# udaysankar01/xfeatSLAM

Measured on AMD Instinct MI355X. Metric: XFeat frames/s (VGA, 4096 kpts) + 4096x4096 desc-match pairs/s, higher is better.
Workload: dtype f32

## Files before the change

### xfeatslam_amd/csrc/kernels_conv.hip

```cpp
#include "ctx.h"
#include "heads_kp4.hip.h"
#include <stdlib.h>

struct ConvArgs {
    const float* in;
    StatSrc st;
    size_t in_stride;
    int Hin, Win;
    const float* w;
    const float* bias;
    float* out;
    size_t out_stride;
    int Hout, Wout;
    double* part;
    size_t part_stride;
    int tiles_x;
    const float* pool; size_t pool_stride; const float* skip_w; const float* skip_b;
    const float* r4; size_t s4; int H4, W4; StatSrc st4;
    const float* r5; size_t s5; int H5, W5; StatSrc st5;
    const float* xstat; const float* w0; const float* bias0;
    int dbg;
};

enum { PRO_PLAIN = 0, PRO_BN = 1, PRO_IN = 2, PRO_B2IN = 3, PRO_FUSE = 4, PRO_L0 = 5, PRO_UNFOLD = 6, PRO_FUSEA = 7  };
// ... 364 lines not shown
                                              int rows_left, int cols_left, int co0, int h, const float (&bias)[NT] ,
                                              double (&sum)[NT], double (&sq)[NT]) {
    static_assert(WW >= 8 && WW * WH == 32, "pixel block of a wave");
    XFH_MFMA_SETTLE();
    const bool full = rows_left >= WH && cols_left >= WW;
    const int lane_off = 4 * h * COUT + co0;
    const int rowstride = Wout * COUT;
    auto value = [&](int n, int r, float* dst, float bv) {
        float v = acc[n][r];
        if constexpr (EPI != EPI_STATS) v += bv;
        if constexpr (EPI == EPI_BIAS_RELU) v = fmaxf(v, 0.f);
        dst[lane_off] = v;
        if constexpr (EPI == EPI_STATS) { const double dv = (double)v; sum[n] += dv; sq[n] = fma(dv, dv, sq[n]); }
    };
    if (full) {
#pragma unroll
        for (int n = 0; n < NT; ++n) {
            sum[n] = 0.0; sq[n] = 0.0;
            if (COUT % 32 == 0 || co0 + n * 32 < COUT) {
#pragma unroll
                for (int r = 0; r < 16; ++r) {
                    const int pb = (r & 3) + 8 * (r >> 2);
                    value(n, r, wave_out + (pb / WW) * rowstride + (pb % WW) * COUT + n * 32, bias[n]);
                }
            }
        }
        return;
    }
#pragma unroll
    for (int n = 0; n < NT; ++n) {
        const int co = co0 + n * 32;
        sum[n] = 0.0; sq[n] = 0.0;
        const float bv = bias[n];
        const bool cok = COUT % 32 == 0 || co < COUT;
#pragma unroll
        for (int r = 0; r < 16; ++r) {
            const int pb = (r & 3) + 8 * (r >> 2);
            const int prow = pb / WW, pcol = pb % WW;
            float* dst = wave_out + prow * rowstride + pcol * COUT + n * 32;
            if (cok && prow < rows_left && pcol + 4 * h < cols_left) value(n, r, dst, bv);
        }
    }
}

#ifndef XFH_PD
#define XFH_PD 3
#endif

template <int CIN, int COUT, int KS, int ST, int WM, int WN, int NT, int WW, int PRO, int EPI, int CBMAX = 64, int TPC = 1, int PD = XFH_PD>
__device__ __forceinline__ void conv_mfma_body(const ConvArgs a, const int tile, const int b, float* smem) {
    constexpr int NTHR = 64 * WM * WN;
    constexpr int WH = 32 / WW, TH = WM * WH, TW = WW;
    constexpr int COUTP = WN * NT * 32;
    constexpr int PAD = KS / 2;
    constexpr int TIH = (TH - 1) * ST + KS, TIW = (TW - 1) * ST + KS;
    constexpr int CP = CIN + 4;
    constexpr int CB = CIN > CBMAX ? CBMAX : CIN;
    constexpr int NCB = CIN / CB;
    static_assert(TPC == 1 || NCB == 1, "several taps per chunk only with all channels in the chunk");
    static_assert((KS * KS) % TPC == 0, "taps per chunk");
    constexpr int NCHUNK = KS * KS * NCB / TPC;
    constexpr int NWBUF = NCHUNK > 1 ? 2 : 1;
    constexpr int KC = TPC * CB;
    constexpr int WS = KC + 4;
    constexpr int WCH = COUTP * KC;
    constexpr int NWLD = (WCH / 4 + NTHR - 1) / NTHR;
    constexpr int G = CIN / 8;
    constexpr int IN_FLOATS = TIH * TIW * CP;
    constexpr int W_FLOATS = COUTP * WS;

    float* s_in = smem;
    float* s_w = smem + IN_FLOATS;
    float* s_stat = s_w + NWBUF * W_FLOATS;

    const int t = threadIdx.x;
    const int tx0 = (tile % a.tiles_x) * TW, ty0 = (tile / a.tiles_x) * TH;
    const float* in = a.in + (size_t)b * a.in_stride;

    XFH_STAMP(a, 0);
    f32x4 wreg[PD][NWLD];
    const __amdgpu_buffer_rsrc_t wrs = wbuf_make(a.w);
#pragma unroll
    for (int c = 0; c < PD; ++c)
#pragma unroll
        for (int q = 0; q < NWLD; ++q) {
            const int f = t + q * NTHR;
            if (c < NCHUNK && f < WCH / 4) wreg[c][q] = wbuf_ld(wrs, f, c * WCH);
        }
    constexpr int NITEM = TIH * TIW * G;
    constexpr int NIT = (NITEM + NTHR - 1) / NTHR;
    constexpr bool FUSE = PRO == PRO_FUSE || PRO == PRO_FUSEA;
    constexpr bool BATCHED = !FUSE;
    f32x4 r0[BATCHED ? NIT : 1], r1[BATCHED ? NIT : 1];
    float rp[PRO == PRO_B2IN ? NIT : 1];
    if constexpr (BATCHED) {
#pragma unroll
        for (int k = 0; k < NIT; ++k) {
            const int item = t + k * NTHR, pix = item / G, g = item % G;
            const int gy = min(max(ty0 * ST - PAD + pix / TIW, 0), a.Hin - 1), gx = min(max(tx0 * ST - PAD + pix % TIW, 0), a.Win - 1);
            const float* p = PRO == PRO_UNFOLD ? in + ((size_t)(gy * 8 + g) * (a.Win * 8) + gx * 8) : in + ((size_t)gy * a.Win + gx) * CIN + g * 8;
            r0[k] = *(const f32x4*)p;
            r1[k] = *(const f32x4*)(p + 4);
            if constexpr (PRO == PRO_B2IN) rp[k] = a.pool[(size_t)b * a.pool_stride + (size_t)gy * a.Win + gx];
        }
    }
    XFH_STAMP(a, 1);
    if constexpr (PRO == PRO_BN || PRO == PRO_B2IN || FUSE) stage_stat(a.st, b, CIN, tile == 0, s_stat, (double*)s_in, t, NTHR);
    if constexpr (PRO == PRO_B2IN) {
        for (int q = t; q < CIN; q += NTHR) { s_stat[2 * CIN + q] = a.skip_w[q]; s_stat[3 * CIN + q] = a.skip_b[q]; }
        __syncthreads();
    }
    if constexpr (PRO == PRO_FUSE) {
        stage_stat(a.st4, b, 64, tile == 0, s_stat + 128, (double*)s_in, t, NTHR);
        stage_stat(a.st5, b, 64, tile == 0, s_stat + 256, (double*)s_in, t, NTHR);
    }
    XFH_STAMP(a, 2);
    if constexpr (BATCHED) {
#pragma unroll
        for (int k = 0; k < NIT; ++k) {
            const int item = t + k * NTHR, pix = item / G, g = item % G;
            const int gy = ty0 * ST - PAD + pix / TIW, gx = tx0 * ST - PAD + pix % TIW;
            const bool ok = gy >= 0 && gy < a.Hin && gx >= 0 && gx < a.Win;
            if (NITEM % NTHR != 0 && item >= NITEM) continue;
            f32x4 v0 = r0[k], v1 = r1[k];
            if constexpr (PRO == PRO_UNFOLD) {
                const float xm = a.xstat[b * 2], xr = a.xstat[b * 2 + 1];
#pragma unroll
                for (int q = 0; q < 4; ++q) { v0[q] = fmaf(v0[q], xr, xm); v1[q] = fmaf(v1[q], xr, xm); }
            }
            if constexpr (PRO == PRO_BN || PRO == PRO_B2IN) {
                const f32x4 m0 = *(const f32x4*)(s_stat + g * 8), m1 = *(const f32x4*)(s_stat + g * 8 + 4);
                const f32x4 q0 = *(const f32x4*)(s_stat + CIN + g * 8), q1 = *(const f32x4*)(s_stat + CIN + g * 8 + 4);
#pragma unroll
                for (int q = 0; q < 4; ++q) {
                    v0[q] = fmaxf(fmaf(v0[q], q0[q], m0[q]), 0.f);
                    v1[q] = fmaxf(fmaf(v1[q], q1[q], m1[q]), 0.f);
                }
            }
            if constexpr (PRO == PRO_B2IN) {
                const float pl = rp[k];
#pragma unroll
                for (int q = 0; q < 4; ++q) {
                    v0[q] = v0[q] + (pl * s_stat[2 * CIN + g * 8 + q] + s_stat[3 * CIN + g * 8 + q]);
                    v1[q] = v1[q] + (pl * s_stat[2 * CIN + g * 8 + 4 + q] + s_stat[3 * CIN + g * 8 + 4 + q]);
                }
            }
            if constexpr (KS > 1) { if (!ok) { v0 = f32x4{0.f, 0.f, 0.f, 0.f}; v1 = v0; } }
            float* d = s_in + pix * CP + g * 8;
            *(f32x4*)d = f32x4{v0.x, v0.z, v1.x, v1.z};
            *(f32x4*)(d + 4) = f32x4{v0.y, v0.w, v1.y, v1.w};
        }
    } else
    for (int item = t; item < TIH * TIW * G; item += NTHR) {
        const int pix = item / G, g = item % G;
        const int iy = pix / TIW, ix = pix % TIW;
        const int gy = ty0 * ST - PAD + iy, gx = tx0 * ST - PAD + ix;
        f32x4 v0 = {0.f, 0.f, 0.f, 0.f}, v1 = {0.f, 0.f, 0.f, 0.f};
        if (gy >= 0 && gy < a.Hin && gx >= 0 && gx < a.Win) {
            const float* p = in + ((size_t)gy * a.Win + gx) * CIN + g * 8;
            v0 = *(const f32x4*)p;
            v1 = *(const f32x4*)(p + 4);
#pragma unroll
            for (int q = 0; q < 4; ++q) {
                v0[q] = fmaxf(fmaf(v0[q], s_stat[CIN + g * 8 + q], s_stat[g * 8 + q]), 0.f);
                v1[q] = fmaxf(fmaf(v1[q], s_stat[CIN + g * 8 + 4 + q], s_stat[g * 8 + 4 + q]), 0.f);
            }
            f32x4 u0, u1, w0, w1;
            up_bilinear8<PRO == PRO_FUSEA>(a.r4 + (size_t)b * a.s4, s_stat + 128, a.H4, a.W4, a.Hin, a.Win, gy, gx, g, u0, u1);
            up_bilinear8<PRO == PRO_FUSEA>(a.r5 + (size_t)b * a.s5, s_stat + 256, a.H5, a.W5, a.Hin, a.Win, gy, gx, g, w0, w1);
#pragma unroll
            for (int q = 0; q < 4; ++q) { v0[q] = (v0[q] + u0[q]) + w0[q]; v1[q] = (v1[q] + u1[q]) + w1[q]; }
        }
        float* d = s_in + pix * CP + g * 8;
        *(f32x4*)d = f32x4{v0.x, v0.z, v1.x, v1.z};
        *(f32x4*)(d + 4) = f32x4{v0.y, v0.w, v1.y, v1.w};
    }
#pragma unroll
    for (int q = 0; q < NWLD; ++q) {
        const int f = t + q * NTHR;
        if (f < WCH / 4) {
            const int n = f / (KC / 4), c4 = f % (KC / 4);
            *(f32x4*)(s_w + n * WS + c4 * 4) = wreg[0][q];
            if (PD < NCHUNK) wreg[0][q] = wbuf_ld(wrs, f, PD * WCH);
        }
    }
    __syncthreads();
    XFH_STAMP(a, 3);

    const int wave = __builtin_amdgcn_readfirstlane(t >> 6), lane = t & 63, i = lane & 31, h = lane >> 5;
    const int wm = wave / WN, wn = wave % WN;
    const int pr = i / WW, pc = i % WW;
    const int ly = (wm * WH + pr) * ST, lx = pc * ST;

    float biasv[NT];
    conv_bias<COUT, NT, EPI>(a.bias, wn * NT * 32 + i, biasv);
    f32x16 acc[NT];
#pragma unroll
    for (int n = 0; n < NT; ++n)
#pragma unroll
        for (int r = 0; r < 16; ++r) acc[n][r] = 0.f;

#pragma unroll
    for (int ch = 0; ch < NCHUNK; ++ch) {
#pragma unroll
        for (int tt = 0; tt < TPC; ++tt) {
            const int tap = TPC == 1 ? ch / NCB : ch * TPC + tt, cb = TPC == 1 ? ch % NCB : 0;
            const int ky = tap / KS, kx = tap % KS;
            const float* pa = s_in + ((ly + ky) * TIW + lx + kx) * CP + cb * CB + 4 * h;
            const float* pw = s_w + (ch & 1) * W_FLOATS + (wn * NT * 32 + i) * WS + tt * CB + 4 * h;
#pragma unroll
            for (int kk = 0; kk < CB / 8; ++kk) {
                const f32x4 av = *(const f32x4*)(pa + kk * 8);
#pragma unroll
                for (int n = 0; n < NT; ++n) {
                    const f32x4 bv = *(const f32x4*)(pw + n * 32 * WS + kk * 8);
#pragma unroll
                    for (int j = 0; j < 4; ++j)
                        acc[n] = __builtin_amdgcn_mfma_f32_32x32x2f32(av[j], bv[j], acc[n], 0, 0, 0);
                }
            }
        }
        if (ch + 1 < NCHUNK) {
            float* wd = s_w + ((ch + 1) & 1) * W_FLOATS;
#pragma unroll
            for (int q = 0; q < NWLD; ++q) {
                const int f = t + q * NTHR;
                if (f < WCH / 4) {
                    const int n = f / (KC / 4), c4 = f % (KC / 4);
                    *(f32x4*)(wd + n * WS + c4 * 4) = wreg[(ch + 1) % PD][q];
                    if (ch + 1 + PD < NCHUNK) wreg[(ch + 1) % PD][q] = wbuf_ld(wrs, f, (ch + 1 + PD) * WCH);
                }
            }
        }
        __syncthreads();
    }

    XFH_STAMP(a, 4);
    double sum[NT], sq[NT];
    {
        const int oy0 = ty0 + wm * WH;
        float* wave_out = a.out + (size_t)b * a.out_stride + ((size_t)oy0 * a.Wout + tx0) * COUT;
        conv_epilogue<COUT, NT, WW, WH, EPI>(acc, wave_out, a.Wout, a.Hout - oy0, a.Wout - tx0, wn * NT * 32 + i, h, biasv, sum, sq);
    }
    if constexpr (EPI == EPI_STATS) {
        double* s_red = (double*)smem;
#pragma unroll
        for (int n = 0; n < NT; ++n) {
            sum[n] += __shfl_xor(sum[n], 32);
            sq[n] += __shfl_xor(sq[n], 32);
            if (h == 0) {
                const int co = (wn * NT + n) * 32 + i;
                s_red[(wm * COUTP + co) * 2 + 0] = sum[n];
                s_red[(wm * COUTP + co) * 2 + 1] = sq[n];
            }
        }
        __syncthreads();
        for (int co = t; co < COUT; co += NTHR) {
            double S = 0.0, SS = 0.0;
#pragma unroll
            for (int m = 0; m < WM; ++m) { S += s_red[(m * COUTP + co) * 2 + 0]; SS += s_red[(m * COUTP + co) * 2 + 1]; }
            double* p = a.part + (size_t)b * a.part_stride + ((size_t)tile * COUT + co) * 2;
            p[0] = S; p[1] = SS;
        }
    }
    XFH_STAMP(a, 5);
}

template <int CIN, int COUT, int KS, int ST, int WM, int WN, int NT, int WW, int PRO, int EPI, int CBMAX = 64, int TPC = 1, int PD = XFH_PD>
__global__ __launch_bounds__(64 * WM * WN)
void k_conv_mfma(ConvArgs a) {
    extern __shared__ __attribute__((aligned(16))) float smem[];
    conv_mfma_body<CIN, COUT, KS, ST, WM, WN, NT, WW, PRO, EPI, CBMAX, TPC, PD>(a, blockIdx.x, blockIdx.z, smem);
}

enum { RIDE_UNFOLD = 0 , RIDE_BN = 1 , RIDE_KP4 = 2  };
template <int CIN, int COUT, int KS, int ST, int WM, int WN, int NT, int WW, int PRO, int CBMAX, int TPC, int RIDER, int EPI = EPI_STATS>
__global__ __launch_bounds__(256)
void k_conv_mfma_ride(ConvArgs a, int n_host, ConvArgs r, Kp4Args k) {
    static_assert(WM * WN == 4, "256 threads");
    extern __shared__ __attribute__((aligned(16))) float smem[];
    const int blk = blockIdx.x;
    if (blk < n_host) conv_mfma_body<CIN, COUT, KS, ST, WM, WN, NT, WW, PRO, EPI, CBMAX, TPC>(a, blk, blockIdx.z, smem);
    else if constexpr (RIDER == RIDE_KP4) { if (threadIdx.x < 4 * HK4_PX) heads_kp4_body(k, blk - n_host, blockIdx.z, smem); }
    else conv_mfma_body<64, 64, 1, 1, 4, 1, 2, 16, RIDER == RIDE_UNFOLD ? PRO_UNFOLD : PRO_BN, EPI>(r, blk - n_host, blockIdx.z, smem);
}

template <int CIN, int COUT, int KS, int ST, int WM, int WN, int NT, int WW, int PRO, int EPI>
__global__ __launch_bounds__(64 * WM * WN)
void k_conv_mfma_p(ConvArgs a, int ntile, int total) {
    constexpr int NTHR = 64 * WM * WN;
    constexpr int WH = 32 / WW, TH = WM * WH, TW = WW;
    constexpr int COUTP = WN * NT * 32;
    constexpr int PAD = KS / 2;
    constexpr int TIH = (TH - 1) * ST + KS, TIW = (TW - 1) * ST + KS;
    constexpr int CP = CIN + 4;
    constexpr int KTOT = KS * KS * CIN;
    constexpr int WS = KTOT + 4;
    constexpr int G = CIN / 8;
    constexpr int NITEM = TIH * TIW * G;
    constexpr int NE = NTHR / G * G;
    constexpr int NIT = (NITEM + NE - 1) / NE;
    constexpr int IN_FLOATS = TIH * TIW * CP;
    constexpr int W_FLOATS = COUTP * WS;
    static_assert(NIT <= 32, "inside mask");

    extern __shared__ __attribute__((aligned(16))) float smem[];
    float* s_in = smem;
    float* s_w = smem + IN_FLOATS;
    double* s_red = (double*)(s_w + W_FLOATS);

    const int t = threadIdx.x;
    for (int f = t; f < COUTP * (KTOT / 4); f += NTHR) {
        const int n = f / (KTOT / 4), c4 = f % (KTOT / 4);
        *(f32x4*)(s_w + n * WS + c4 * 4) = *(const f32x4*)(a.w + (size_t)f * 4);
    }
    const int g = t % G;
    const int wave = __builtin_amdgcn_readfirstlane(t >> 6), lane = t & 63, i = lane & 31, h = lane >> 5;
    const int wm = wave / WN, wn = wave % WN;
    const int pr = i / WW, pc = i % WW;
    const int ly = (wm * WH + pr) * ST, lx = pc * ST;

    f32x4 v0[NIT], v1[NIT];
    float pl[NIT];
    unsigned inside = 0u;
    auto load_tile = [&](int tile) {
        const int b = tile / ntile, tl = tile - b * ntile;
        const int tx0 = (tl % a.tiles_x) * TW, ty0 = (tl / a.tiles_x) * TH;
        const float* in = a.in + (size_t)b * a.in_stride + (PRO == PRO_UNFOLD ? 0 : g * 8);
        inside = 0u;
#pragma unroll
        for (int k = 0; k < NIT; ++k) {
            const int item = t + k * NE;
            const int pix = item / G;
            const int iy = pix / TIW, ix = pix % TIW;
            const int gy = ty0 * ST - PAD + iy, gx = tx0 * ST - PAD + ix;
            if constexpr (KS == 1) {
                const int cy = min(max(gy, 0), a.Hin - 1), cx = min(max(gx, 0), a.Win - 1);
                const float* p = PRO == PRO_UNFOLD ? in + ((cy * 8 + g) * (a.Win * 8) + cx * 8) : in + (cy * a.Win + cx) * CIN;
                v0[k] = *(const f32x4*)p; v1[k] = *(const f32x4*)(p + 4);
            } else {
                v0[k] = f32x4{0.f, 0.f, 0.f, 0.f}; v1[k] = v0[k];
                if (t < NE && item < NITEM && gy >= 0 && gy < a.Hin && gx >= 0 && gx < a.Win) {
                    const float* p = in + (gy * a.Win + gx) * CIN;
                    v0[k] = *(const f32x4*)p; v1[k] = *(const f32x4*)(p + 4);
                    if constexpr (PRO == PRO_B2IN) pl[k] = a.pool[(size_t)b * a.pool_stride + (size_t)gy * a.Win + gx];
                    inside |= 1u << k;
                }
            }
        }
    };
    auto store_tile = [&](int tile) {
        f32x4 m0, m1, r0, r1, w0, w1, c0, c1;
        if constexpr (PRO == PRO_BN || PRO == PRO_B2IN) {
            const int b = tile / ntile;
            const float* st = a.st.stat + (size_t)b * 2 * CIN + g * 8;
            m0 = *(const f32x4*)st; m1 = *(const f32x4*)(st + 4); r0 = *(const f32x4*)(st + CIN); r1 = *(const f32x4*)(st + CIN + 4);
        }
        if constexpr (PRO == PRO_B2IN) {
            w0 = *(const f32x4*)(a.skip_w + g * 8); w1 = *(const f32x4*)(a.skip_w + g * 8 + 4);
            c0 = *(const f32x4*)(a.skip_b + g * 8); c1 = *(const f32x4*)(a.skip_b + g * 8 + 4);
        }
#pragma unroll
        for (int k = 0; k < NIT; ++k) {
            const int item = t + k * NE;
            if (t < NE && item < NITEM) {
                f32x4 x0 = v0[k], x1 = v1[k];
                [[maybe_unused]] const bool in_img = inside & (1u << k);
                if constexpr (KS == 1) {
                    float xm = 0.f, xr = 1.f;
                    if constexpr (PRO == PRO_UNFOLD) { const int fb = tile / ntile; xm = a.xstat[fb * 2]; xr = a.xstat[fb * 2 + 1]; }
#pragma unroll
                    for (int q = 0; q < 4; ++q) {
                        if constexpr (PRO == PRO_UNFOLD) { x0[q] = fmaf(x0[q], xr, xm); x1[q] = fmaf(x1[q], xr, xm); }
                        if constexpr (PRO == PRO_BN) {
                            x0[q] = fmaxf(fmaf(x0[q], r0[q], m0[q]), 0.f);
                            x1[q] = fmaxf(fmaf(x1[q], r1[q], m1[q]), 0.f);
                        }
                    }
                } else if constexpr (PRO == PRO_BN || PRO == PRO_B2IN) {
                    if (in_img) {
#pragma unroll
                        for (int q = 0; q < 4; ++q) {
                            x0[q] = fmaxf(fmaf(x0[q], r0[q], m0[q]), 0.f);
                            x1[q] = fmaxf(fmaf(x1[q], r1[q], m1[q]), 0.f);
                            if constexpr (PRO == PRO_B2IN) { x0[q] = x0[q] + (pl[k] * w0[q] + c0[q]); x1[q] = x1[q] + (pl[k] * w1[q] + c1[q]); }
                        }
                    }
                }
                float* d = s_in + (item / G) * CP + g * 8;
                *(f32x4*)d = f32x4{x0.x, x0.z, x1.x, x1.z};
                *(f32x4*)(d + 4) = f32x4{x0.y, x0.w, x1.y, x1.w};
            }
        }
    };

    int tile = blockIdx.x;
    if (tile >= total) return;
    float biasv[NT];
    conv_bias<COUT, NT, EPI>(a.bias, wn * NT * 32 + i, biasv);
    load_tile(tile);
    store_tile(tile);
    __syncthreads();
    while (true) {
        const int next = tile + gridDim.x;
        const bool has_next = next < total;
        if (has_next) load_tile(next);

        f32x16 acc[NT];
#pragma unroll
        for (int n = 0; n < NT; ++n)
#pragma unroll
            for (int r = 0; r < 16; ++r) acc[n][r] = 0.f;
#pragma unroll
        for (int tap = 0; tap < KS * KS; ++tap) {
            const int ky = tap / KS, kx = tap % KS;
            const float* pa = s_in + ((ly + ky) * TIW + lx + kx) * CP + 4 * h;
            const float* pw = s_w + (wn * NT * 32 + i) * WS + tap * CIN + 4 * h;
#pragma unroll
            for (int kk = 0; kk < CIN / 8; ++kk) {
                const f32x4 av = *(const f32x4*)(pa + kk * 8);
#pragma unroll
                for (int n = 0; n < NT; ++n) {
                    const f32x4 bv = *(const f32x4*)(pw + n * 32 * WS + kk * 8);
#pragma unroll
                    for (int j = 0; j < 4; ++j)
                        acc[n] = __builtin_amdgcn_mfma_f32_32x32x2f32(av[j], bv[j], acc[n], 0, 0, 0);
                }
            }
        }

        const int b = tile / ntile, tl = tile - b * ntile;
        const int tx0 = (tl % a.tiles_x) * TW, ty0 = (tl / a.tiles_x) * TH;
        double sum[NT], sq[NT];
        {
            const int oy0 = ty0 + wm * WH;
            float* wave_out = a.out + (size_t)b * a.out_stride + ((size_t)oy0 * a.Wout + tx0) * COUT;
            conv_epilogue<COUT, NT, WW, WH, EPI>(acc, wave_out, a.Wout, a.Hout - oy0, a.Wout - tx0, wn * NT * 32 + i, h, biasv, sum, sq);
        }
        if constexpr (EPI == EPI_STATS) {
#pragma unroll
            for (int n = 0; n < NT; ++n) {
                sum[n] += __shfl_xor(sum[n], 32);
                sq[n] += __shfl_xor(sq[n], 32);
                if (h == 0) {
                    const int co = (wn * NT + n) * 32 + i;
                    s_red[(wm * COUTP + co) * 2 + 0] = sum[n];
                    s_red[(wm * COUTP + co) * 2 + 1] = sq[n];
                }
            }
        }
        __syncthreads();
        if constexpr (EPI == EPI_STATS) {
            for (int co = t; co < COUT; co += NTHR) {
                double S = 0.0, SS = 0.0;
#pragma unroll
                for (int m = 0; m < WM; ++m) { S += s_red[(m * COUTP + co) * 2 + 0]; SS += s_red[(m * COUTP + co) * 2 + 1]; }
                double* p = a.part + (size_t)b * a.part_stride + ((size_t)tl * COUT + co) * 2;
                p[0] = S; p[1] = SS;
            }
        }
        if (!has_next) break;
        store_tile(next);
        __syncthreads();
        tile = next;
    }
}

template <int CIN, int COUT, int KS, int ST, int WM, int WN, int NT, int WW, int PRO, int EPI, int CBMAX = 64>
__global__ __launch_bounds__(64 * WM * WN)
void k_conv_mfma_t(ConvArgs a, int ntile, int total) {
    static_assert(PRO == PRO_BN, "layers behind a finalised BatchNorm (large batches)");
    constexpr int NTHR = 64 * WM * WN;
    constexpr int WH = 32 / WW, TH = WM * WH, TW = WW;
    constexpr int COUTP = WN * NT * 32;
    constexpr int PAD = KS / 2;
    constexpr int TIH = (TH - 1) * ST + KS, TIW = (TW - 1) * ST + KS;
    constexpr int CP = CIN + 4;
    constexpr int CB = CIN > CBMAX ? CBMAX : CIN;
    constexpr int NCB = CIN / CB;
    constexpr int NCHUNK = KS * KS * NCB;
    static_assert(NCHUNK >= 3 && NCHUNK % 3 == 0, "the chunk ring (three LDS buffers, three register sets) closes on itself");
    constexpr int WS = CB + 4;
    constexpr int WCH = COUTP * CB;
    constexpr int NWLD = (WCH / 4 + NTHR - 1) / NTHR;
    constexpr int G = CIN / 8;
    constexpr int NITEM = TIH * TIW * G;
    constexpr int NE = NTHR / G * G;
    constexpr int NIT = (NITEM + NE - 1) / NE;
    constexpr int IN_FLOATS = TIH * TIW * CP;
    constexpr int W_FLOATS = COUTP * WS;
    static_assert(NIT <= 32, "inside mask");
    constexpr int SPC = CB / 8;
    constexpr int GS = (NT == 1 && SPC % 2 == 0) ? 2 : 1;
    constexpr int GPC = SPC / GS, NGT = NCHUNK * GPC;

    extern __shared__ __attribute__((aligned(16))) float smem[];
    float* s_in = smem;
    float* s_w = smem + IN_FLOATS;
    double* s_red = (double*)(s_w + 3 * W_FLOATS);

    const int t = threadIdx.x;
    const int g = t % G;
    const int wave = __builtin_amdgcn_readfirstlane(t >> 6), lane = t & 63, i = lane & 31, h = lane >> 5;
    const int wm = wave / WN, wn = wave % WN;
    const int pr = i / WW, pc = i % WW;
    const int ly = (wm * WH + pr) * ST, lx = pc * ST;

    int tile = blockIdx.x;
    if (tile >= total) return;
    f32x4 wreg[3][NWLD];
    const __amdgpu_buffer_rsrc_t wrs = wbuf_make(a.w);
#pragma unroll
    for (int c = 0; c < 3; ++c)
#pragma unroll
        for (int q = 0; q < NWLD; ++q) {
            const int f = t + q * NTHR;
            if (f < WCH / 4) wreg[c][q] = wbuf_ld(wrs, f, c * WCH);
        }

    f32x4 v0[NIT], v1[NIT], m0, m1, r0, r1;
    unsigned inside = 0u;
    auto load_tile = [&](int tl_) {
        const int b = tl_ / ntile, tl = tl_ - b * ntile;
        const int tx0 = (tl % a.tiles_x) * TW, ty0 = (tl / a.tiles_x) * TH;
        const float* in = a.in + (size_t)b * a.in_stride + g * 8;
        inside = 0u;
#pragma unroll
        for (int k = 0; k < NIT; ++k) {
            const int item = t + k * NE;
            const int pix = (NITEM % NE != 0 && k == NIT - 1) ? min(item, NITEM - 1) / G : item / G;
            const int gy = ty0 * ST - PAD + pix / TIW, gx = tx0 * ST - PAD + pix % TIW;
            const int cy = min(max(gy, 0), a.Hin - 1), cx = min(max(gx, 0), a.Win - 1);
            const float* p = in + ((size_t)cy * a.Win + cx) * CIN;
            v0[k] = *(const f32x4*)p; v1[k] = *(const f32x4*)(p + 4);
            inside |= (gy == cy && gx == cx) ? (1u << k) : 0u;
        }
        const float* st = a.st.stat + (size_t)b * 2 * CIN + g * 8;
        m0 = *(const f32x4*)st; m1 = *(const f32x4*)(st + 4); r0 = *(const f32x4*)(st + CIN); r1 = *(const f32x4*)(st + CIN + 4);
    };
    auto store_tile = [&]() {
#pragma unroll
        for (int k = 0; k < NIT; ++k) {
            const int item = t + k * NE;
            if (t < NE && item < NITEM) {
                f32x4 x0 = v0[k], x1 = v1[k];
                const bool in_img = inside & (1u << k);
#pragma unroll
                for (int q = 0; q < 4; ++q) {
                    x0[q] = fmaxf(fmaf(x0[q], r0[q], m0[q]), 0.f);
                    x1[q] = fmaxf(fmaf(x1[q], r1[q], m1[q]), 0.f);
                    x0[q] = in_img ? x0[q] : 0.f; x1[q] = in_img ? x1[q] : 0.f;
                }
                float* d = s_in + (item / G) * CP + g * 8;
                *(f32x4*)d = f32x4{x0.x, x0.z, x1.x, x1.z};
                *(f32x4*)(d + 4) = f32x4{x0.y, x0.w, x1.y, x1.w};
            }
        }
    };
    auto push_chunk = [&](int rc) {
        float* wd = s_w + (rc % 3) * W_FLOATS;
        const int wsrc_off = ((rc + 3) % NCHUNK) * WCH;
#pragma unroll
        for (int q = 0; q < NWLD; ++q) {
            const int f = t + q * NTHR;
            if (f < WCH / 4) {
                const int n = f / (CB / 4), c4 = f % (CB / 4);
                *(f32x4*)(wd + n * WS + c4 * 4) = wreg[rc % 3][q];
                wreg[rc % 3][q] = wbuf_ld(wrs, f, wsrc_off);
            }
        }
    };

    float biasv[NT];
    conv_bias<COUT, NT, EPI>(a.bias, wn * NT * 32 + i, biasv);
    load_tile(tile);
    store_tile();
    push_chunk(0);
    push_chunk(1);
    __syncthreads();

    f32x4 av[2][GS], bv[2][GS][NT];
    auto load_group = [&](int q, int buf) {
#pragma unroll
        for (int u = 0; u < GS; ++u) {
            const int ch = q / GPC, kk = (q % GPC) * GS + u;
            const int tap = ch / NCB, cb = ch % NCB;
            const int ky = tap / KS, kx = tap % KS;
            av[buf][u] = *(const f32x4*)(s_in + ((ly + ky) * TIW + lx + kx) * CP + cb * CB + 4 * h + kk * 8);
#pragma unroll
            for (int n = 0; n < NT; ++n)
                bv[buf][u][n] = *(const f32x4*)(s_w + (ch % 3) * W_FLOATS + (wn * NT * 32 + i + n * 32) * WS + 4 * h + kk * 8);
        }
    };
    while (true) {
        const int next = tile + gridDim.x;
        const bool has_next = next < total;
        f32x16 acc[NT];
        auto mfma_part = [&](int buf, int part, bool first) {
            if constexpr (GS == 2) {
#pragma unroll
                for (int n = 0; n < NT; ++n)
#pragma unroll
                    for (int j = 0; j < 4; ++j) acc[n] = __builtin_amdgcn_mfma_f32_32x32x2f32(av[buf][part][j], bv[buf][part][n][j], acc[n], 0, 0, 0);
            } else {
#pragma unroll
                for (int j = 2 * part; j < 2 * part + 2; ++j)
#pragma unroll
                    for (int n = 0; n < NT; ++n) acc[n] = __builtin_amdgcn_mfma_f32_32x32x2f32(av[buf][0][j], bv[buf][0][n][j], acc[n], 0, 0, 0);
            }
        };
#pragma unroll
        for (int n = 0; n < NT; ++n)
#pragma unroll
            for (int r = 0; r < 16; ++r) acc[n][r] = 0.f;
        load_group(0, 0);
        push_chunk(2);
        if (has_next) load_tile(next);
#pragma unroll
        for (int q = 0; q < NGT; ++q) {
            const int cur = q & 1;
            if (q > 0 && q % GPC == 0) {
                __builtin_amdgcn_s_waitcnt(0xc07f);
                __builtin_amdgcn_s_barrier();
                push_chunk(q / GPC + 2);
            }
            __builtin_amdgcn_sched_barrier(0);
            mfma_part(cur, 0, q == 0);
            __builtin_amdgcn_sched_barrier(0);
            if (q + 1 < NGT) load_group(q + 1, cur ^ 1);
            __builtin_amdgcn_sched_barrier(0);
            mfma_part(cur, 1, false);
            __builtin_amdgcn_sched_barrier(0);
        }

        const int b = tile / ntile, tl = tile - b * ntile;
        const int tx0 = (tl % a.tiles_x) * TW, ty0 = (tl / a.tiles_x) * TH;
        double sum[NT], sq[NT];
        {
            const int oy0 = ty0 + wm * WH;
            float* wave_out = a.out + (size_t)b * a.out_stride + ((size_t)oy0 * a.Wout + tx0) * COUT;
            conv_epilogue<COUT, NT, WW, WH, EPI>(acc, wave_out, a.Wout, a.Hout - oy0, a.Wout - tx0, wn * NT * 32 + i, h, biasv, sum, sq);
        }
        if constexpr (EPI == EPI_STATS) {
#pragma unroll
            for (int n = 0; n < NT; ++n) {
                sum[n] += __shfl_xor(sum[n], 32);
                sq[n] += __shfl_xor(sq[n], 32);
                if (h == 0) {
                    const int co = (wn * NT + n) * 32 + i;
                    s_red[(wm * COUTP + co) * 2 + 0] = sum[n];
                    s_red[(wm * COUTP + co) * 2 + 1] = sq[n];
                }
            }
        }
        __syncthreads();
        if constexpr (EPI == EPI_STATS) {
            for (int co = t; co < COUT; co += NTHR) {
                double S = 0.0, SS = 0.0;
#pragma unroll
                for (int m = 0; m < WM; ++m) { S += s_red[(m * COUTP + co) * 2 + 0]; SS += s_red[(m * COUTP + co) * 2 + 1]; }
                double* p = a.part + (size_t)b * a.part_stride + ((size_t)tl * COUT + co) * 2;
                p[0] = S; p[1] = SS;
            }
        }
        if (!has_next) break;
        store_tile();
        __syncthreads();
        tile = next;
    }
}

template <int CIN, int COUT, int ST, int GW, int PGY, int PRO, int EPI, int PD = 3, int CGS = 1>
__global__ __launch_bounds__(64 * PGY * (COUT / 16 / CGS))
void k_conv_mfma16(ConvArgs a) {
    static_assert(PRO == PRO_BN || PRO == PRO_FUSE, "3x3 layers behind a BatchNorm (block_fusion.0: + the pyramid sum)");
    constexpr int GH = 16 / GW, CG = COUT / 16 / CGS, COUTW = CG * 16, NW = PGY * CG, NTHR = 64 * NW;
    static_assert(COUT % (16 * CGS) == 0, "channel split");
    constexpr int TH = GH * PGY, TW = GW, TIH = (TH - 1) * ST + 3, TIW = (TW - 1) * ST + 3, CP = CIN + 4;
    constexpr int CB = 64, NCB = CIN / CB, NCHUNK = 9 * NCB, KC = CB, WS = KC + 4;
    constexpr int WCH = COUT * KC , WCW = COUTW * KC , NWLD = (WCW / 4 + NTHR - 1) / NTHR;
    constexpr int G = CIN / 8, NITEM = TIH * TIW * G, NIT = (NITEM + NTHR - 1) / NTHR;
    constexpr int IN_FLOATS = TIH * TIW * CP, W_FLOATS = COUTW * WS;
    static_assert(sizeof(double) * 512 <= sizeof(float) * IN_FLOATS, "bn_fold scratch in the input tile");
    static_assert(sizeof(double) * PGY * COUTW * 2 <= sizeof(float) * IN_FLOATS, "statistics scratch in the input tile");

    extern __shared__ __attribute__((aligned(16))) float smem[];
    float* s_in = smem;
    float* s_w = smem + IN_FLOATS;
    float* s_stat = s_w + 3 * W_FLOATS;

    constexpr int FB = NTHR > 512 ? 8 : 16;
    const int t = threadIdx.x, b = blockIdx.z;
    const int tile = blockIdx.x, tx0 = (tile % a.tiles_x) * TW, ty0 = (tile / a.tiles_x) * TH;
    const float* in = a.in + (size_t)b * a.in_stride;
    const int co0 = blockIdx.y * COUTW;
    const float* wg = a.w + (size_t)co0 * KC;
    const __amdgpu_buffer_rsrc_t wrs = wbuf_make(wg);

    XFH_STAMP(a, 0);
    f32x4 wreg[PD][NWLD];
#pragma unroll
    for (int c = 0; c < PD; ++c)
#pragma unroll
        for (int q = 0; q < NWLD; ++q) {
            const int f = t + q * NTHR;
            if (c < NCHUNK && f < WCW / 4) wreg[c][q] = wbuf_ld(wrs, f, c * WCH);
        }
    f32x4 r0[NIT], r1[NIT];
#pragma unroll
    for (int k = 0; k < NIT; ++k) {
        const int item = t + k * NTHR, pix = item / G, g = item % G;
        const int gy = min(max(ty0 * ST - 1 + pix / TIW, 0), a.Hin - 1), gx = min(max(tx0 * ST - 1 + pix % TIW, 0), a.Win - 1);
        const float* p = in + ((size_t)gy * a.Win + gx) * CIN + g * 8;
        r0[k] = *(const f32x4*)p;
        r1[k] = *(const f32x4*)(p + 4);
    }
    XFH_STAMP(a, 1);
    stage_stat<FB>(a.st, b, CIN, tile == 0, s_stat, (double*)s_in, t, NTHR);
    if constexpr (PRO == PRO_FUSE) {
        stage_stat<FB>(a.st4, b, 64, tile == 0, s_stat + 128, (double*)s_in, t, NTHR);
        stage_stat<FB>(a.st5, b, 64, tile == 0, s_stat + 256, (double*)s_in, t, NTHR);
    }
    XFH_STAMP(a, 2);
#pragma unroll
    for (int k = 0; k < NIT; ++k) {
        const int item = t + k * NTHR, pix = item / G, g = item % G;
        const int gy = ty0 * ST - 1 + pix / TIW, gx = tx0 * ST - 1 + pix % TIW;
        const bool ok = gy >= 0 && gy < a.Hin && gx >= 0 && gx < a.Win;
        if (NITEM % NTHR != 0 && item >= NITEM) continue;
        f32x4 v0 = r0[k], v1 = r1[k];
        const f32x4 m0 = *(const f32x4*)(s_stat + g * 8), m1 = *(const f32x4*)(s_stat + g * 8 + 4);
        const f32x4 q0 = *(const f32x4*)(s_stat + CIN + g * 8), q1 = *(const f32x4*)(s_stat + CIN + g * 8 + 4);
#pragma unroll
        for (int e = 0; e < 4; ++e) {
            v0[e] = fmaxf(fmaf(v0[e], q0[e], m0[e]), 0.f);
            v1[e] = fmaxf(fmaf(v1[e], q1[e], m1[e]), 0.f);
        }
        if constexpr (PRO == PRO_FUSE) {
            const int cy = min(max(gy, 0), a.Hin - 1), cx = min(max(gx, 0), a.Win - 1);
            f32x4 u0, u1, w0, w1;
            up_bilinear8(a.r4 + (size_t)b * a.s4, s_stat + 128, a.H4, a.W4, a.Hin, a.Win, cy, cx, g, u0, u1);
            if constexpr (NTHR > 512) __builtin_amdgcn_sched_barrier(0);
            up_bilinear8(a.r5 + (size_t)b * a.s5, s_stat + 256, a.H5, a.W5, a.Hin, a.Win, cy, cx, g, w0, w1);
#pragma unroll
            for (int e = 0; e < 4; ++e) { v0[e] = (v0[e] + u0[e]) + w0[e]; v1[e] = (v1[e] + u1[e]) + w1[e]; }
        }
        if (!ok) { v0 = f32x4{0.f, 0.f, 0.f, 0.f}; v1 = v0; }
        float* d = s_in + pix * CP + (g >> 1) * 16 + 2 * (g & 1);
#pragma unroll
        for (int e = 0; e < 4; ++e) *(f32x2*)(d + 4 * e) = f32x2{v0[e], v1[e]};
    }
    static_assert(PD >= 2 && NCHUNK >= 3, "two chunks go to LDS before the loop");
#pragma unroll
    for (int c = 0; c < 2; ++c)
#pragma unroll
        for (int q = 0; q < NWLD; ++q) {
            const int f = t + q * NTHR;
            if (f < WCW / 4) {
                const int n = f / (KC / 4), c4 = f % (KC / 4);
                *(f32x4*)(s_w + c * W_FLOATS + n * WS + c4 * 4) = wreg[c][q];
                if (c + PD < NCHUNK) wreg[c][q] = wbuf_ld(wrs, f, (c + PD) * WCH);
            }
        }
    __syncthreads();
    XFH_STAMP(a, 3);

// ... 677 lines not shown
```

Baseline: 31990.

## Use buffer loads with precomputed offsets and stage next tile before epilogue

For KS>1 convs, per-item pixel offsets are precomputed once and input loads use raw buffer loads with an out-of-range offset for padding, so bounds checks are skipped on interior tiles. BN stats and skip weights are hoisted out of the per-tile store. The next tile is written to LDS right after the MFMA loop, behind an extra barrier, so staging overlaps the epilogue's global writes. This adds a barrier per tile and more live registers, and depends on buffer OOB returning zeros.

```diff
diff --git a/xfeatslam_amd/csrc/kernels_conv.hip b/xfeatslam_amd/csrc/kernels_conv.hip
--- a/xfeatslam_amd/csrc/kernels_conv.hip
+++ b/xfeatslam_amd/csrc/kernels_conv.hip
@@ -690,7 +690,6 @@
     constexpr int NIT = (NITEM + NE - 1) / NE;
     constexpr int IN_FLOATS = TIH * TIW * CP;
     constexpr int W_FLOATS = COUTP * WS;
-    static_assert(NIT <= 32, "inside mask");
 
     extern __shared__ __attribute__((aligned(16))) float smem[];
     float* s_in = smem;
@@ -710,50 +709,82 @@
 
     f32x4 v0[NIT], v1[NIT];
     float pl[NIT];
-    unsigned inside = 0u;
+    constexpr int NG = KS == 1 ? 1 : NIT;
+    constexpr unsigned OOB = 0x80000000u;
+    int sy[NG], sx[NG];
+    unsigned soff[NG], spoff[NG];
+    bool ok[NG];
+    bool interior = true;
+    f32x4 m0, m1, r0, r1, w0, w1, c0, c1;
+    if constexpr (KS > 1) {
+#pragma unroll
+        for (int k = 0; k < NIT; ++k) {
+            const int item = t + k * NE;
+            const int pix = (t < NE && item < NITEM) ? item / G : 0;
+            sy[k] = pix / TIW; sx[k] = pix % TIW;
+            const int po = sy[k] * a.Win + sx[k];
+            soff[k] = (unsigned)(po * CIN + g * 8) * 4u;
+            spoff[k] = (unsigned)po * 4u;
+            ok[k] = true;
+        }
+        if constexpr (PRO == PRO_B2IN) {
+            w0 = *(const f32x4*)(a.skip_w + g * 8); w1 = *(const f32x4*)(a.skip_w + g * 8 + 4);
+            c0 = *(const f32x4*)(a.skip_b + g * 8); c1 = *(const f32x4*)(a.skip_b + g * 8 + 4);
+        }
+    }
     auto load_tile = [&](int tile) {
         const int b = tile / ntile, tl = tile - b * ntile;
         const int tx0 = (tl % a.tiles_x) * TW, ty0 = (tl / a.tiles_x) * TH;
-        const float* in = a.in + (size_t)b * a.in_stride + (PRO == PRO_UNFOLD ? 0 : g * 8);
-        inside = 0u;
-#pragma unroll
-        for (int k = 0; k < NIT; ++k) {
-            const int item = t + k * NE;
-            const int pix = item / G;
-            const int iy = pix / TIW, ix = pix % TIW;
-            const int gy = ty0 * ST - PAD + iy, gx = tx0 * ST - PAD + ix;
-            if constexpr (KS == 1) {
+        if constexpr (KS == 1) {
+            const float* in = a.in + (size_t)b * a.in_stride + (PRO == PRO_UNFOLD ? 0 : g * 8);
+#pragma unroll
+            for (int k = 0; k < NIT; ++k) {
+                const int item = t + k * NE;
+                const int pix = item / G;
+                const int iy = pix / TIW, ix = pix % TIW;
+                const int gy = ty0 * ST - PAD + iy, gx = tx0 * ST - PAD + ix;
                 const int cy = min(max(gy, 0), a.Hin - 1), cx = min(max(gx, 0), a.Win - 1);
                 const float* p = PRO == PRO_UNFOLD ? in + ((cy * 8 + g) * (a.Win * 8) + cx * 8) : in + (cy * a.Win + cx) * CIN;
                 v0[k] = *(const f32x4*)p; v1[k] = *(const f32x4*)(p + 4);
-            } else {
-                v0[k] = f32x4{0.f, 0.f, 0.f, 0.f}; v1[k] = v0[k];
-                if (t < NE && item < NITEM && gy >= 0 && gy < a.Hin && gx >= 0 && gx < a.Win) {
-                    const float* p = in + (gy * a.Win + gx) * CIN;
-                    v0[k] = *(const f32x4*)p; v1[k] = *(const f32x4*)(p + 4);
-                    if constexpr (PRO == PRO_B2IN) pl[k] = a.pool[(size_t)b * a.pool_stride + (size_t)gy * a.Win + gx];
-                    inside |= 1u << k;
-                }
+            }
+        } else {
+            const int y0 = ty0 * ST - PAD, x0 = tx0 * ST - PAD;
+            interior = y0 >= 0 && y0 + TIH <= a.Hin && x0 >= 0 && x0 + TIW <= a.Win;
+            const ptrdiff_t o0 = (ptrdiff_t)y0 * a.Win + x0;
+            const __amdgpu_buffer_rsrc_t rin = wbuf_make(a.in + ((ptrdiff_t)b * a.in_stride + o0 * CIN));
+            [[maybe_unused]] const __amdgpu_buffer_rsrc_t rpl = wbuf_make(PRO == PRO_B2IN ? a.pool + ((ptrdiff_t)b * a.pool_stride + o0) : a.in);
+#pragma unroll
+            for (int k = 0; k < NIT; ++k) {
+                unsigned oi = soff[k], op = spoff[k];
+                bool in_img = true;
+                if (!interior) {
+                    in_img = (unsigned)(y0 + sy[k]) < (unsigned)a.Hin && (unsigned)(x0 + sx[k]) < (unsigned)a.Win;
+                    if (!in_img) { oi = OOB; op = OOB; }
+                }
+                ok[k] = in_img;
+                v0[k] = __builtin_bit_cast(f32x4, __builtin_amdgcn_raw_buffer_load_b128(rin, oi, 0, 0));
+                v1[k] = __builtin_bit_cast(f32x4, __builtin_amdgcn_raw_buffer_load_b128(rin, oi + 16u, 0, 0));
+                if constexpr (PRO == PRO_B2IN) pl[k] = __builtin_bit_cast(float, __builtin_amdgcn_raw_buffer_load_b32(rpl, op, 0, 0));
+            }
+            if constexpr (PRO == PRO_BN || PRO == PRO_B2IN) {
+                const float* st = a.st.stat + (size_t)b * 2 * CIN + g * 8;
+                m0 = *(const f32x4*)st; m1 = *(const f32x4*)(st + 4); r0 = *(const f32x4*)(st + CIN); r1 = *(const f32x4*)(st + CIN + 4);
             }
         }
     };
     auto store_tile = [&](int tile) {
-        f32x4 m0, m1, r0, r1, w0, w1, c0, c1;
-        if constexpr (PRO == PRO_BN || PRO == PRO_B2IN) {
-            const int b = tile / ntile;
-            const float* st = a.st.stat + (size_t)b * 2 * CIN + g * 8;
-            m0 = *(const f32x4*)st; m1 = *(const f32x4*)(st + 4); r0 = *(const f32x4*)(st + CIN); r1 = *(const f32x4*)(st + CIN + 4);
-        }
-        if constexpr (PRO == PRO_B2IN) {
-            w0 = *(const f32x4*)(a.skip_w + g * 8); w1 = *(const f32x4*)(a.skip_w + g * 8 + 4);
-            c0 = *(const f32x4*)(a.skip_b + g * 8); c1 = *(const f32x4*)(a.skip_b + g * 8 + 4);
+        if constexpr (KS == 1) {
+            if constexpr (PRO == PRO_BN) {
+                const int b = tile / ntile;
+                const float* st = a.st.stat + (size_t)b * 2 * CIN + g * 8;
+                m0 = *(const f32x4*)st; m1 = *(const f32x4*)(st + 4); r0 = *(const f32x4*)(st + CIN); r1 = *(const f32x4*)(st + CIN + 4);
+            }
         }
 #pragma unroll
         for (int k = 0; k < NIT; ++k) {
             const int item = t + k * NE;
             if (t < NE && item < NITEM) {
                 f32x4 x0 = v0[k], x1 = v1[k];
-                [[maybe_unused]] const bool in_img = inside & (1u << k);
                 if constexpr (KS == 1) {
                     float xm = 0.f, xr = 1.f;
                     if constexpr (PRO == PRO_UNFOLD) { const int fb = tile / ntile; xm = a.xstat[fb * 2]; xr = a.xstat[fb * 2 + 1]; }
@@ -765,8 +796,8 @@
                             x1[q] = fmaxf(fmaf(x1[q], r1[q], m1[q]), 0.f);
                         }
                     }
-                } else if constexpr (PRO == PRO_BN || PRO == PRO_B2IN) {
-                    if (in_img) {
+                } else {
+                    if constexpr (PRO == PRO_BN || PRO == PRO_B2IN) {
 #pragma unroll
                         for (int q = 0; q < 4; ++q) {
                             x0[q] = fmaxf(fmaf(x0[q], r0[q], m0[q]), 0.f);
@@ -774,6 +805,7 @@
                             if constexpr (PRO == PRO_B2IN) { x0[q] = x0[q] + (pl[k] * w0[q] + c0[q]); x1[q] = x1[q] + (pl[k] * w1[q] + c1[q]); }
                         }
                     }
+                    if (!interior && !ok[k]) { x0 = f32x4{0.f, 0.f, 0.f, 0.f}; x1 = x0; }
                 }
                 float* d = s_in + (item / G) * CP + g * 8;
                 *(f32x4*)d = f32x4{x0.x, x0.z, x1.x, x1.z};
@@ -817,6 +849,12 @@
             }
         }
 
+        constexpr bool STAGE_FIRST = KS > 1;
+        if constexpr (STAGE_FIRST) {
+            __syncthreads();
+            if (has_next) store_tile(next);
+        }
+
         const int b = tile / ntile, tl = tile - b * ntile;
         const int tx0 = (tl % a.tiles_x) * TW, ty0 = (tl / a.tiles_x) * TH;
         double sum[NT], sq[NT];
@@ -848,8 +886,10 @@
             }
         }
         if (!has_next) break;
-        store_tile(next);
-        __syncthreads();
+        if constexpr (!STAGE_FIRST) {
+            store_tile(next);
+            __syncthreads();
+        }
         tile = next;
     }
 }
```

Result: faster. 32490 (median of 6 runs) (+1.6%).
